# tomer-erez/Psychoacoustic-adverserial-attacks

Measured on AMD Instinct MI355X. Metric: pgd_steps_per_sec, higher is better.
Workload: dtype bf16x3 (split-bf16 hi+lo, three MFMA passes, f32 accumulate: fp32-parity); 1 GPU; untargeted PGD, norm_type snr snr_db 40, Wav2Vec2-base (rule-generated weights), 32x10s 16 kHz clips per GPU, 150-token labels; global_batch=32, per_gpu_batch=32, samples_per_clip=160000, parallelism=dp1, hip_graph=True, hip_graph_replayed_steps=80

## Files before the change

psychoacoustic-adverserial-attacks_amd/build_ext.py:

```python
from __future__ import annotations

import hashlib
import os
import subprocess
import sys
from concurrent.futures import ThreadPoolExecutor

HERE = os.path.dirname(os.path.abspath(__file__))
CSRC = os.path.join(HERE, "csrc")
INCLUDE = os.path.join(os.path.dirname(HERE), "include")
SOURCES = ["proj_kernels.hip", "spec_kernels.hip", "mask_kernels.hip", "gemm.hip", "gemm_ring.hip", "gemm_ring2.hip", "model_kernels.hip", "conv0_dgrad.hip", "attention.hip", "model.hip", "wer_kernels.hip", "place_kernels.hip", "rir_kernels.hip", "chan_kernels.hip", "search_kernels.hip", "eot_kernels.hip"]
FLAGS = ["-O3", "--offload-arch=gfx950", "-fPIC", "-std=c++17", "-Wno-unused-value"] + os.environ.get("PAA_EXTRA_HIPCC_FLAGS", "").split()
VARIANT = "_exp" if os.environ.get("PAA_EXTRA_HIPCC_FLAGS", "").strip() else ""
LIB = os.path.join(HERE, f"libpaa_hip{VARIANT}.so")


def _hipcc() -> str:
    for c in (os.environ.get("HIPCC"), "/opt/rocm/bin/hipcc", "hipcc"):
        if c and (os.path.isabs(c) and os.path.exists(c) or not os.path.isabs(c)):
            return c
    return "hipcc"


def _digest(paths, extra=()) -> str:
    h = hashlib.sha256()
    for x in extra:
        h.update(str(x).encode() + b"\0")
    for p in sorted(paths):
        h.update(os.path.basename(p).encode() + b"\0")
        with open(p, "rb") as f:
            h.update(f.read())
        h.update(b"\0")
    return h.hexdigest()


def _headers():
    out = [os.path.join(CSRC, f) for f in os.listdir(CSRC) if f.endswith(".h")]
    out += [os.path.join(INCLUDE, f) for f in os.listdir(INCLUDE) if f.endswith(".h")]
    return out


def source_key() -> str:
    files = [os.path.join(CSRC, f) for f in os.listdir(CSRC) if f.endswith((".hip", ".h"))]
    files += [os.path.join(INCLUDE, f) for f in os.listdir(INCLUDE) if f.endswith(".h")]
    return _digest(files, FLAGS + SOURCES)


def _read(path):
    try:
        with open(path) as f:
            return f.read().strip()
    except OSError:
        return None


def is_current() -> bool:
    return os.path.exists(LIB) and _read(LIB + ".key") == source_key()


def build(force: bool = False, verbose: bool = True) -> str:
    key = source_key()
    if not force and os.path.exists(LIB) and _read(LIB + ".key") == key:
        return LIB
    objdir = os.path.join(HERE, "build" + VARIANT)
    os.makedirs(objdir, exist_ok=True)
    hipcc = _hipcc()
    hdrs = _headers()

    def cc(src):
        obj = os.path.join(objdir, src.replace(".hip", ".o"))
        okey = _digest([os.path.join(CSRC, src)] + hdrs, FLAGS)
        if not force and os.path.exists(obj) and _read(obj + ".key") == okey:
            return obj
        cmd = [hipcc, *FLAGS, "-c", os.path.join(CSRC, src), "-o", obj]
        if verbose:
            print(" ".join(cmd), flush=True)
        r = subprocess.run(cmd, capture_output=True, text=True)
        if r.returncode != 0:
            raise RuntimeError(f"hipcc failed on {src}:\n{r.stdout}\n{r.stderr}")
        with open(obj + ".key", "w") as f:
            f.write(okey)
        return obj

    with ThreadPoolExecutor(max_workers=4) as ex:
        objs = list(ex.map(cc, SOURCES))
    cmd = [hipcc, "--offload-arch=gfx950", "-shared", "-fPIC", "-o", LIB, *objs]
    if verbose:
        print(" ".join(cmd), flush=True)
    r = subprocess.run(cmd, capture_output=True, text=True)
    if r.returncode != 0:
        raise RuntimeError(f"link failed:\n{r.stdout}\n{r.stderr}")
    with open(LIB + ".key", "w") as f:
        f.write(key)
    return LIB


if __name__ == "__main__":
    print(build(force="--force" in sys.argv))
```

psychoacoustic-adverserial-attacks_amd/csrc/gemm.hip:

```cpp
#include <algorithm>
#include <vector>

#include "gemm_dev.h"

namespace paa {

template <int ROWS, bool IS_A>
__device__ __forceinline__ void load_kc(const paa_gemm_desc& d, const float* __restrict__ base, int64_t ld, int r0,
                                        int k0, int rlim, float4 (&v)[ROWS / 32]) {
    const int tid = threadIdx.x;
    const int k = k0 + ((tid & 7) << 2);
    int64_t koff = k;
    int js = 0, kc = k;
    if (IS_A && d.a_kseg > 0) {
        js = k / d.a_kseg;
        kc = k - js * d.a_kseg;
        koff = (int64_t)js * d.a_kseg_stride + kc;
    }
#pragma unroll
    for (int i = 0; i < ROWS / 32; ++i) {
        const int r = r0 + (tid >> 3) + 32 * i;
        float4 x = make_float4(0.f, 0.f, 0.f, 0.f);
        bool ok = (r < rlim) && (k < d.K);
        const float* p;
        if (IS_A && d.a_window) {
            const int tr = r + js - d.a_pad;
            ok = ok && (tr >= 0) && (tr < d.a_rows_valid);
            p = base + (int64_t)tr * ld + kc;
        } else {
            p = base + (int64_t)r * ld + koff;
        }
        if (ok) {
            x = *reinterpret_cast<const float4*>(p);
            if (k + 3 >= d.K) {
                if (k + 1 >= d.K) x.y = 0.f;
                if (k + 2 >= d.K) x.z = 0.f;
                x.w = 0.f;
            }
        }
        v[i] = x;
    }
}

template <int ROWS>
__device__ __forceinline__ void load_rc(const paa_gemm_desc& d, const float* __restrict__ base, int64_t ld, int r0,
                                        int k0, int rlim, float4 (&v)[ROWS / 32]) {
    constexpr int VPK = ROWS / 4;
    constexpr int KSTEP = G_NT / VPK;
    const int tid = threadIdx.x;
    const int r = r0 + ((tid % VPK) << 2);
#pragma unroll
    for (int i = 0; i < ROWS / 32; ++i) {
        const int k = k0 + tid / VPK + KSTEP * i;
        float4 x = make_float4(0.f, 0.f, 0.f, 0.f);
        if (k < d.K && r < rlim) {
            x = *reinterpret_cast<const float4*>(base + (int64_t)k * ld + r);
            if (r + 3 >= rlim) {
                if (r + 1 >= rlim) x.y = 0.f;
                if (r + 2 >= rlim) x.z = 0.f;
                x.w = 0.f;
            }
        }
        v[i] = x;
    }
}

template <int ROWS, int PREC>
__device__ __forceinline__ void store_kc(unsigned short* hi, unsigned short* lo, const float4 (&v)[ROWS / 32]) {
    const int tid = threadIdx.x;
#pragma unroll
    for (int i = 0; i < ROWS / 32; ++i) {
        const int off = ((tid >> 3) + 32 * i) * G_LD + ((tid & 7) << 2);
        const float f[4] = {v[i].x, v[i].y, v[i].z, v[i].w};
        unsigned short h[4], l[4];
#pragma unroll
        for (int j = 0; j < 4; ++j) {
            h[j] = bf16_bits(f[j]);
            if (PREC) l[j] = bf16_bits(f[j] - bf16_to_f32(h[j]));
        }
        *reinterpret_cast<uint2*>(hi + off) = make_uint2(h[0] | ((unsigned)h[1] << 16), h[2] | ((unsigned)h[3] << 16));
        if (PREC)
            *reinterpret_cast<uint2*>(lo + off) = make_uint2(l[0] | ((unsigned)l[1] << 16), l[2] | ((unsigned)l[3] << 16));
    }
}

template <int ROWS, int PREC>
__device__ __forceinline__ void store_rc(unsigned short* hi, unsigned short* lo, const float4 (&v)[ROWS / 32]) {
    constexpr int VPK = ROWS / 4;
    constexpr int KSTEP = G_NT / VPK;
    const int tid = threadIdx.x;
#pragma unroll
    for (int i = 0; i < ROWS / 32; ++i) {
        const int k = tid / VPK + KSTEP * i;
        const int r = (tid % VPK) << 2;
        const float f[4] = {v[i].x, v[i].y, v[i].z, v[i].w};
#pragma unroll
        for (int j = 0; j < 4; ++j) {
            const unsigned short h = bf16_bits(f[j]);
            hi[(r + j) * G_LD + k] = h;
            if (PREC) lo[(r + j) * G_LD + k] = bf16_bits(f[j] - bf16_to_f32(h));
        }
    }
}

template <int BN, int PREC, bool AKC, bool BKC>
__global__ __launch_bounds__(G_NT) void k_gemm(GemmArgs g) {
    constexpr int NPL = PREC ? 2 : 1;
    constexpr int NJ = BN / 64;
    __shared__ __attribute__((aligned(16))) unsigned short smem[NPL * (G_BM + BN) * G_LD];
    unsigned short* sAh = smem;
    unsigned short* sAl = smem + (PREC ? G_BM * G_LD : 0);
    unsigned short* sBh = smem + NPL * G_BM * G_LD;
    unsigned short* sBl = sBh + (PREC ? BN * G_LD : 0);

    const paa_gemm_desc& d = g.d;
    const int nwg = g.tiles_m * g.tiles_n;
    const int orig = blockIdx.x;
    const int q = nwg >> 3, r8 = nwg & 7, xcd = orig & 7;
    const int id = (xcd < r8 ? xcd * (q + 1) : r8 * (q + 1) + (xcd - r8) * q) + (orig >> 3);
    const int tm = id / g.tiles_n, tn = id - tm * g.tiles_n;
    const int m0 = tm * G_BM, n0 = tn * BN;
    const int z = blockIdx.y;
    const int z1 = z / d.batch2, z2 = z - z1 * d.batch2;
    const float* A = d.A + z1 * d.a_s1 + z2 * d.a_s2;
    const float* B = d.B + z1 * d.b_s1 + z2 * d.b_s2;

    const int tid = threadIdx.x, lane = tid & 63, wave = tid >> 6;
    const int wm = wave >> 1, wn = wave & 1;
    const int lr = lane & 31, lh = lane >> 5;

    f32x16 acc[2][NJ];
#pragma unroll
    for (int i = 0; i < 2; ++i)
#pragma unroll
        for (int j = 0; j < NJ; ++j)
#pragma unroll
            for (int e = 0; e < 16; ++e) acc[i][j][e] = 0.f;

    float4 ra[G_BM / 32], rb[BN / 32];
    const int nk = (d.K + G_BK - 1) / G_BK;
    if (AKC) load_kc<G_BM, true>(d, A, d.lda, m0, 0, d.M, ra); else load_rc<G_BM>(d, A, d.lda, m0, 0, d.M, ra);
    if (BKC) load_kc<BN, false>(d, B, d.ldb, n0, 0, d.N, rb); else load_rc<BN>(d, B, d.ldb, n0, 0, d.N, rb);

    for (int kt = 0; kt < nk; ++kt) {
        if (AKC) store_kc<G_BM, PREC>(sAh, sAl, ra); else store_rc<G_BM, PREC>(sAh, sAl, ra);
        if (BKC) store_kc<BN, PREC>(sBh, sBl, rb); else store_rc<BN, PREC>(sBh, sBl, rb);
        __syncthreads();
        if (kt + 1 < nk) {
            const int k0 = (kt + 1) * G_BK;
            if (AKC) load_kc<G_BM, true>(d, A, d.lda, m0, k0, d.M, ra); else load_rc<G_BM>(d, A, d.lda, m0, k0, d.M, ra);
            if (BKC) load_kc<BN, false>(d, B, d.ldb, n0, k0, d.N, rb); else load_rc<BN>(d, B, d.ldb, n0, k0, d.N, rb);
        }
#pragma unroll
        for (int ks = 0; ks < 2; ++ks) {
            bf16x8 ah[2], al[2], bh[NJ], bl[NJ];
#pragma unroll
            for (int i = 0; i < 2; ++i) {
                const int off = (wm * 64 + i * 32 + lr) * G_LD + ks * 16 + lh * 8;
                ah[i] = *reinterpret_cast<const bf16x8*>(sAh + off);
                if (PREC) al[i] = *reinterpret_cast<const bf16x8*>(sAl + off);
            }
#pragma unroll
            for (int j = 0; j < NJ; ++j) {
                const int off = (wn * (BN / 2) + j * 32 + lr) * G_LD + ks * 16 + lh * 8;
                bh[j] = *reinterpret_cast<const bf16x8*>(sBh + off);
                if (PREC) bl[j] = *reinterpret_cast<const bf16x8*>(sBl + off);
            }
#pragma unroll
            for (int i = 0; i < 2; ++i)
#pragma unroll
                for (int j = 0; j < NJ; ++j) {
                    if (PREC) {
                        acc[i][j] = __builtin_amdgcn_mfma_f32_32x32x16_bf16(al[i], bh[j], acc[i][j], 0, 0, 0);
                        acc[i][j] = __builtin_amdgcn_mfma_f32_32x32x16_bf16(ah[i], bl[j], acc[i][j], 0, 0, 0);
                    }
                    acc[i][j] = __builtin_amdgcn_mfma_f32_32x32x16_bf16(ah[i], bh[j], acc[i][j], 0, 0, 0);
                }
        }
        __syncthreads();
    }

    epilogue<NJ, 2>(d, acc, m0 + wm * 64 + 4 * lh, n0 + wn * (BN / 2) + lr, z1, z2);
}

constexpr int H_BK = 64, H_LD = 72;

template <int ROWS, bool IS_A, int NT>
__device__ __forceinline__ void load_bf(const paa_gemm_desc& d, const unsigned short* __restrict__ base, int64_t ld,
                                        int r0, int k0, int rlim, uint4 (&v)[ROWS * 8 / NT], int tid, int il = 0) {
    const int k = k0 + ((tid & 7) << 3);
    int64_t koff = il ? ((k >> 5) << 6) + (k & 31) + (il == 2 ? 32 : 0) : k;
    int js = 0, kc = k;
    if (IS_A && d.a_kseg > 0) {
        js = k / d.a_kseg;
        kc = k - js * d.a_kseg;
        koff = (int64_t)js * d.a_kseg_stride + kc;
    }
#pragma unroll
    for (int i = 0; i < ROWS * 8 / NT; ++i) {
        const int r = r0 + (tid >> 3) + (NT / 8) * i;
        uint4 x = make_uint4(0u, 0u, 0u, 0u);
        bool ok = (r < rlim) && (k < d.K);
        const unsigned short* p;
        if (IS_A && d.a_window) {
            const int tr = r + js - d.a_pad;
            ok = ok && (tr >= 0) && (tr < d.a_rows_valid);
            p = base + (int64_t)tr * ld + kc;
        } else {
            p = base + (int64_t)r * ld + koff;
        }
        if (ok) x = *reinterpret_cast<const uint4*>(p);
        v[i] = x;
    }
}

typedef unsigned int u32x4 __attribute__((ext_vector_type(4)));
__device__ __forceinline__ __amdgpu_buffer_rsrc_t tile_rsrc(const unsigned short* base, int64_t elems) {
    const int64_t bytes = elems > 0 ? 2 * elems : 0;
    return __builtin_amdgcn_make_buffer_rsrc(const_cast<unsigned short*>(base), 0,
                                             (int)(unsigned)(bytes > 0xFFFFFFFFll ? 0xFFFFFFFFll : bytes), 0x00020000);
}
template <int ROWS, int NT>
__device__ __forceinline__ void load_buf(__amdgpu_buffer_rsrc_t rs, unsigned voff, unsigned k0_bytes, unsigned step_bytes,
                                         uint4 (&v)[ROWS * 8 / NT]) {
#pragma unroll
    for (int i = 0; i < ROWS * 8 / NT; ++i) {
        const u32x4 x = __builtin_amdgcn_raw_buffer_load_b128(rs, voff, k0_bytes + i * step_bytes, 0);
        v[i] = make_uint4(x.x, x.y, x.z, x.w);
    }
}

template <int ROWS, int NT, bool PERM, bool SWZ = false>
__device__ __forceinline__ void store_bf(unsigned short* lds, const uint4 (&v)[ROWS * 8 / NT], int tid) {
    constexpr int LD = SWZ ? 64 : H_LD;
#pragma unroll
    for (int i = 0; i < ROWS * 8 / NT; ++i) {
        int r = (tid >> 3) + (NT / 8) * i;
        if (PERM) r = (r & ~63) | ((((r >> 2) & 1) << 5) + (((r & 63) >> 3) << 2) + (r & 3));
        const int ch = SWZ ? ((tid & 7) ^ ((r >> 1) & 7)) : (tid & 7);
        *reinterpret_cast<uint4*>(lds + r * LD + (ch << 3)) = v[i];
    }
}

template <int BM, int BN, int PREC, int WM, bool VEC, bool SEG, bool SWZ = false>
__global__ __launch_bounds__(WM * 128, (WM == 4 && PREC == 0) ? 4 : 2) void k_gemm_bf(GemmArgs g) {
    constexpr int NT = WM * 128;
    constexpr int LD = SWZ ? 64 : H_LD;
    constexpr int NPL = PREC ? 2 : 1;
    constexpr int NJ = BN / 64;
    constexpr int MI = BM / (32 * WM);
    static_assert(!VEC || NJ == 2, "vector epilogue needs 64 columns per wave");
    __shared__ __attribute__((aligned(16))) unsigned short smem[NPL * (BM + BN) * LD];
    unsigned short* sAh = smem;
    unsigned short* sAl = smem + (PREC ? BM * LD : 0);
    unsigned short* sBh = smem + NPL * BM * LD;
    unsigned short* sBl = sBh + (PREC ? BN * LD : 0);

    const paa_gemm_desc& d = g.d;
    const int nwg = g.tiles_m * g.tiles_n;
    const int total = nwg * d.batch;
    const int nk = (d.K + H_BK - 1) / H_BK;
    const int kg_spt = (d.k_group > 0 && d.k_group % H_BK == 0 && d.K % d.k_group == 0 && d.K > d.k_group) ? d.k_group / H_BK : 0;
    const int kg_taps = kg_spt ? d.K / d.k_group : 1;

    struct Tile { int m0, n0, z1, z2; };
    auto decode = [&](int t) {
        Tile c;
        const int z = t / nwg, orig = t - z * nwg;
        const int q = nwg >> 3, r8 = nwg & 7, xcd = orig & 7;
        const int id = (xcd < r8 ? xcd * (q + 1) : r8 * (q + 1) + (xcd - r8) * q) + (orig >> 3);
        const int tm = id / g.tiles_n, tn = id - tm * g.tiles_n;
        c.m0 = tm * BM; c.n0 = tn * BN;
        c.z1 = z / d.batch2; c.z2 = z - c.z1 * d.batch2;
        return c;
    };
    uint4 rah[BM * 8 / NT], rbh[BN * 8 / NT], ral[PREC ? BM * 8 / NT : 1], rbl[PREC ? BN * 8 / NT : 1];
    auto load_tile = [&](const Tile& c, int k0, int tid) {
        const int64_t aoff = c.z1 * d.a_s1 + c.z2 * d.a_s2, boff = c.z1 * d.b_s1 + c.z2 * d.b_s2;
        if constexpr (SEG) {
            const bool ail = PREC && d.A_il != nullptr;
            if (ail) load_bf<BM, true, NT>(d, reinterpret_cast<const unsigned short*>(d.A_il) + 2 * aoff, 2 * d.lda, c.m0, k0, d.M, rah, tid, 1);
            else load_bf<BM, true, NT>(d, reinterpret_cast<const unsigned short*>(d.A) + aoff, d.lda, c.m0, k0, d.M, rah, tid);
            load_bf<BN, false, NT>(d, reinterpret_cast<const unsigned short*>(d.B) + boff, d.ldb, c.n0, k0, d.N, rbh, tid);
            if constexpr (PREC) {
                if (ail) load_bf<BM, true, NT>(d, reinterpret_cast<const unsigned short*>(d.A_il) + 2 * aoff, 2 * d.lda, c.m0, k0, d.M, ral, tid, 2);
                else load_bf<BM, true, NT>(d, reinterpret_cast<const unsigned short*>(d.A_lo) + aoff, d.lda, c.m0, k0, d.M, ral, tid);
                load_bf<BN, false, NT>(d, reinterpret_cast<const unsigned short*>(d.B_lo) + boff, d.ldb, c.n0, k0, d.N, rbl, tid);
            }
        } else if (PREC && d.A_il != nullptr) {
            const int64_t a0 = 2 * aoff + (int64_t)c.m0 * (2 * d.lda), b0 = boff + (int64_t)c.n0 * d.ldb;
            const int64_t ae = (int64_t)(d.M - 1 - c.m0) * (2 * d.lda) + 2 * (int64_t)d.K, be = (int64_t)(d.N - 1 - c.n0) * d.ldb + d.K;
            const unsigned kc = (unsigned)((tid & 7) << 3);
            const unsigned va = 2u * ((unsigned)(tid >> 3) * 2u * (unsigned)d.lda + ((kc >> 5) << 6) + (kc & 31u)), vb = 2u * ((unsigned)(tid >> 3) * (unsigned)d.ldb + kc);
            const unsigned sa = 2u * (NT / 8) * 2u * (unsigned)d.lda, sb = 2u * (NT / 8) * (unsigned)d.ldb;
            const __amdgpu_buffer_rsrc_t ra = tile_rsrc(reinterpret_cast<const unsigned short*>(d.A_il) + a0, ae);
            load_buf<BM, NT>(ra, va, 4u * k0, sa, rah);
            load_buf<BN, NT>(tile_rsrc(reinterpret_cast<const unsigned short*>(d.B) + b0, be), vb, 2u * k0, sb, rbh);
            if constexpr (PREC) {
                load_buf<BM, NT>(ra, va + 64u, 4u * k0, sa, ral);
                load_buf<BN, NT>(tile_rsrc(reinterpret_cast<const unsigned short*>(d.B_lo) + b0, be), vb, 2u * k0, sb, rbl);
            }
        } else {
            const int64_t a0 = aoff + (int64_t)c.m0 * d.lda, b0 = boff + (int64_t)c.n0 * d.ldb;
            const int64_t ae = (int64_t)(d.M - 1 - c.m0) * d.lda + d.K, be = (int64_t)(d.N - 1 - c.n0) * d.ldb + d.K;
            const unsigned kc = (unsigned)((tid & 7) << 3);
            const unsigned va = 2u * ((unsigned)(tid >> 3) * (unsigned)d.lda + kc), vb = 2u * ((unsigned)(tid >> 3) * (unsigned)d.ldb + kc);
            const unsigned sa = 2u * (NT / 8) * (unsigned)d.lda, sb = 2u * (NT / 8) * (unsigned)d.ldb;
            load_buf<BM, NT>(tile_rsrc(reinterpret_cast<const unsigned short*>(d.A) + a0, ae), va, 2u * k0, sa, rah);
            load_buf<BN, NT>(tile_rsrc(reinterpret_cast<const unsigned short*>(d.B) + b0, be), vb, 2u * k0, sb, rbh);
            if constexpr (PREC) {
                load_buf<BM, NT>(tile_rsrc(reinterpret_cast<const unsigned short*>(d.A_lo) + a0, ae), va, 2u * k0, sa, ral);
                load_buf<BN, NT>(tile_rsrc(reinterpret_cast<const unsigned short*>(d.B_lo) + b0, be), vb, 2u * k0, sb, rbl);
            }
        }
    };
    auto store_tile = [&](int tid) {
        store_bf<BM, NT, false, SWZ>(sAh, rah, tid);
        store_bf<BN, NT, VEC, SWZ>(sBh, rbh, tid);
        if constexpr (PREC) { store_bf<BM, NT, false, SWZ>(sAl, ral, tid); store_bf<BN, NT, VEC, SWZ>(sBl, rbl, tid); }
    };

    int t = blockIdx.x;
    if (t >= total) return;
    Tile cur = decode(t);
    load_tile(cur, 0, threadIdx.x);
    store_tile(threadIdx.x);
    for (;;) {
        int tid = threadIdx.x;
        asm volatile("" : "+v"(tid));
        const int lane = tid & 63, wave = tid >> 6;
        const int wm = wave >> 1, wn = wave & 1;
        const int lr = lane & 31, lh = lane >> 5;
        const int tnx = t + gridDim.x;
        const bool more = tnx < total;
        const Tile nxt = more ? decode(tnx) : cur;
        f32x16 acc[MI][NJ];
#pragma unroll
        for (int i = 0; i < MI; ++i)
#pragma unroll
            for (int j = 0; j < NJ; ++j)
#pragma unroll
                for (int e = 0; e < 16; ++e) acc[i][j][e] = 0.f;

        int ktap = 0, kc = 0;
        for (int kt = 0; kt < nk; ++kt) {
            __syncthreads();
            const bool last = kt + 1 == nk;
            int knext = kt + 1;
            if (kg_spt) {
                if (++ktap == kg_taps) { ktap = 0; ++kc; }
                knext = ktap * kg_spt + kc;
            }
            if (!last) load_tile(cur, knext * H_BK, tid);
            else if (more) load_tile(nxt, 0, tid);
            {
                constexpr int KS = H_BK / 16;
                constexpr int NM = NJ * (PREC ? 3 : 1);
                int offk[KS];
#pragma unroll
                for (int q = 0; q < KS; ++q) offk[q] = SWZ ? (((2 * q + lh) ^ ((lr >> 1) & 7)) << 3) : (lh * 8 + q * 16);
                const unsigned short* pa = sAh + (wm * (32 * MI) + lr) * LD;
                const unsigned short* pb = sBh + (wn * (BN / 2) + lr) * LD;
                constexpr int LO_A = BM * LD, LO_B = BN * LD;
                bf16x8 bh[NJ], bl[NJ], bhn[NJ], bln[NJ], ah, al, ahn, aln;
#pragma unroll
                for (int j = 0; j < NJ; ++j) {
                    bh[j] = *reinterpret_cast<const bf16x8*>(pb + j * 32 * LD + offk[0]);
                    if (PREC) bl[j] = *reinterpret_cast<const bf16x8*>(pb + LO_B + j * 32 * LD + offk[0]);
                    bhn[j] = bh[j]; bln[j] = bl[j];
                }
                ah = *reinterpret_cast<const bf16x8*>(pa + offk[0]);
                if (PREC) al = *reinterpret_cast<const bf16x8*>(pa + LO_A + offk[0]);
                ahn = ah; aln = al;
                __builtin_amdgcn_sched_group_barrier(0x100, (NJ + 1) * NPL, 0);
#pragma unroll
                for (int ks = 0; ks < KS; ++ks)
#pragma unroll
                    for (int i = 0; i < MI; ++i) {
                        const int ni = (i + 1 < MI) ? i + 1 : 0, nks = (i + 1 < MI) ? ks : ks + 1;
                        if (nks < KS) {
                            ahn = *reinterpret_cast<const bf16x8*>(pa + ni * 32 * LD + offk[nks < KS ? nks : 0]);
                            if (PREC) aln = *reinterpret_cast<const bf16x8*>(pa + LO_A + ni * 32 * LD + offk[nks < KS ? nks : 0]);
                            if (ni == 0) {
#pragma unroll
                                for (int j = 0; j < NJ; ++j) {
                                    bhn[j] = *reinterpret_cast<const bf16x8*>(pb + j * 32 * LD + offk[nks < KS ? nks : 0]);
                                    if (PREC) bln[j] = *reinterpret_cast<const bf16x8*>(pb + LO_B + j * 32 * LD + offk[nks < KS ? nks : 0]);
                                }
                            }
                        }
#pragma unroll
                        for (int j = 0; j < NJ; ++j) {
                            if (PREC) {
                                acc[i][j] = __builtin_amdgcn_mfma_f32_32x32x16_bf16(al, bh[j], acc[i][j], 0, 0, 0);
                                acc[i][j] = __builtin_amdgcn_mfma_f32_32x32x16_bf16(ah, bl[j], acc[i][j], 0, 0, 0);
                            }
                            acc[i][j] = __builtin_amdgcn_mfma_f32_32x32x16_bf16(ah, bh[j], acc[i][j], 0, 0, 0);
                        }
                        if (nks < KS) {
                            if (ni == 0) __builtin_amdgcn_sched_group_barrier(0x100, (NJ + 1) * NPL, 0);
                            else __builtin_amdgcn_sched_group_barrier(0x100, NPL, 0);
                        }
                        __builtin_amdgcn_sched_group_barrier(0x008, NM, 0);
                        ah = ahn; al = aln;
                        if (ni == 0) {
#pragma unroll
                            for (int j = 0; j < NJ; ++j) { bh[j] = bhn[j]; bl[j] = bln[j]; }
                        }
                    }
            }
            __syncthreads();
            if (!last || more) store_tile(tid);
        }
        {
            int te = tid;
            asm volatile("" : "+v"(te));
            const int el = te & 63, ew = te >> 6;
            if constexpr (VEC) epilogue_vec<MI, true>(d, acc, cur.m0 + (ew >> 1) * (32 * MI), cur.n0 + (ew & 1) * (BN / 2), cur.z1, cur.z2, el);
            else epilogue<NJ, MI>(d, acc, cur.m0 + (ew >> 1) * (32 * MI) + 4 * (el >> 5), cur.n0 + (ew & 1) * (BN / 2) + (el & 31), cur.z1, cur.z2);
        }
        if (!more) break;
        cur = nxt;
        t = tnx;
    }
}

template <int PREC, int KS, int MI, int WV = 4>
__global__ __launch_bounds__(WV * 64, WV == 4 ? 2 : 1) void k_gemm_win(GemmArgs g, int taps) {
    constexpr int NT = WV * 64;
    constexpr int BM = 32 * MI * WV, TB = 4, NPL = PREC ? 2 : 1;
    constexpr int ALD = KS + 8;
    constexpr int BLD = TB * KS + 8;
    constexpr int CPR = KS / 8;
    constexpr int BCH = TB * KS / 8;
    constexpr int NB = (64 * BCH + NT - 1) / NT;
    extern __shared__ __attribute__((aligned(16))) unsigned short smw[];
    const paa_gemm_desc& d = g.d;
    const int srows = BM + taps - 1;
    unsigned short* sA = smw;
    unsigned short* sB = smw + NPL * srows * ALD;
    const int tid = threadIdx.x, lane = tid & 63, wave = tid >> 6, lr = lane & 31, lh = lane >> 5;
    const int m0 = blockIdx.x * BM;
    const int z = blockIdx.y, z1 = z / d.batch2, z2 = z - z1 * d.batch2;
    const int64_t aoff = z1 * d.a_s1 + z2 * d.a_s2, boff = z1 * d.b_s1 + z2 * d.b_s2;
    const unsigned short* Ap[2] = {reinterpret_cast<const unsigned short*>(d.A) + aoff,
                                   PREC ? reinterpret_cast<const unsigned short*>(d.A_lo) + aoff : nullptr};
    const unsigned short* Bp[2] = {reinterpret_cast<const unsigned short*>(d.B) + boff,
                                   PREC ? reinterpret_cast<const unsigned short*>(d.B_lo) + boff : nullptr};
    for (int i = tid; i < srows * CPR; i += NT) {
        const int sr = i / CPR, ch = i - sr * CPR;
        const int tr = m0 - d.a_pad + sr;
        const bool ok = tr >= 0 && tr < d.a_rows_valid;
#pragma unroll
        for (int pl = 0; pl < NPL; ++pl) {
            uint4 x = make_uint4(0u, 0u, 0u, 0u);
            if (ok) x = *reinterpret_cast<const uint4*>(Ap[pl] + (int64_t)tr * d.lda + ch * 8);
            *reinterpret_cast<uint4*>(sA + (pl * srows + sr) * ALD + ch * 8) = x;
        }
    }
    for (int i = tid; i < NPL * 64 * BLD / 8; i += NT) reinterpret_cast<uint4*>(sB)[i] = make_uint4(0u, 0u, 0u, 0u);
    uint4 rb[NPL][NB];
    auto bload = [&](int st) {
#pragma unroll
        for (int u = 0; u < NB; ++u) {
            const int i = tid + NT * u;
            const int n = i / BCH, ch = i - n * BCH;
#pragma unroll
            for (int pl = 0; pl < NPL; ++pl) {
                rb[pl][u] = make_uint4(0u, 0u, 0u, 0u);
                if (i < 64 * BCH && n < d.N) rb[pl][u] = *reinterpret_cast<const uint4*>(Bp[pl] + (int64_t)n * d.ldb + st * (TB * KS) + ch * 8);
            }
        }
    };
    auto bstore = [&]() {
#pragma unroll
        for (int u = 0; u < NB; ++u) {
            const int i = tid + NT * u;
            const int n = i / BCH, ch = i - n * BCH;
            if (i < 64 * BCH && n < d.N) {
#pragma unroll
                for (int pl = 0; pl < NPL; ++pl) *reinterpret_cast<uint4*>(sB + (pl * 64 + n) * BLD + ch * 8) = rb[pl][u];
            }
        }
    };
    __syncthreads();
    bload(0);
    bstore();
    f32x16 acc[MI][2];
#pragma unroll
    for (int i = 0; i < MI; ++i)
#pragma unroll
        for (int j = 0; j < 2; ++j)
#pragma unroll
            for (int e = 0; e < 16; ++e) acc[i][j][e] = 0.f;
    const int nst = taps / TB;
    for (int st = 0; st < nst; ++st) {
        __syncthreads();
        if (st + 1 < nst) bload(st + 1);
        constexpr int NSTEP = TB * (KS / 16);
        const unsigned short* pa0 = sA + (wave * (32 * MI) + lr + st * TB) * ALD + lh * 8;
        const unsigned short* pb0 = sB + lr * BLD + lh * 8;
        bf16x8 ah[2][MI], al[2][MI], bh[2][2], bl[2][2];
        auto fload = [&](int q, int buf) {
            const int tp = q / (KS / 16), ks = q - tp * (KS / 16);
            const unsigned short* pa = pa0 + tp * ALD + ks * 16;
            const unsigned short* pb = pb0 + tp * KS + ks * 16;
#pragma unroll
            for (int i = 0; i < MI; ++i) {
                ah[buf][i] = *reinterpret_cast<const bf16x8*>(pa + i * 32 * ALD);
                if (PREC) al[buf][i] = *reinterpret_cast<const bf16x8*>(pa + (srows + i * 32) * ALD);
            }
#pragma unroll
            for (int j = 0; j < 2; ++j) {
                bh[buf][j] = *reinterpret_cast<const bf16x8*>(pb + j * 32 * BLD);
                if (PREC) bl[buf][j] = *reinterpret_cast<const bf16x8*>(pb + (64 + j * 32) * BLD);
            }
        };
        fload(0, 0);
#pragma unroll
        for (int q = 0; q < NSTEP; ++q) {
            const int cb = q & 1;
            if (q + 1 < NSTEP) fload(q + 1, cb ^ 1);
#pragma unroll
            for (int j = 0; j < 2; ++j)
#pragma unroll
                for (int i = 0; i < MI; ++i) {
                    if (PREC) {
                        acc[i][j] = __builtin_amdgcn_mfma_f32_32x32x16_bf16(al[cb][i], bh[cb][j], acc[i][j], 0, 0, 0);
                        acc[i][j] = __builtin_amdgcn_mfma_f32_32x32x16_bf16(ah[cb][i], bl[cb][j], acc[i][j], 0, 0, 0);
                    }
                    acc[i][j] = __builtin_amdgcn_mfma_f32_32x32x16_bf16(ah[cb][i], bh[cb][j], acc[i][j], 0, 0, 0);
                }
            if constexpr (PREC == 0) {
#pragma unroll
                for (int r = 0; r < (MI + 2 > 2 * MI ? MI + 2 : 2 * MI); ++r) {
                    if (r < 2 * MI) __builtin_amdgcn_sched_group_barrier(0x008, 1, 0);
                    if (r < MI + 2 && q + 1 < NSTEP) __builtin_amdgcn_sched_group_barrier(0x100, 1, 0);
                }
            }
        }
        __syncthreads();
        if (st + 1 < nst) bstore();
    }
    epilogue<2, MI>(d, acc, m0 + wave * (32 * MI) + 4 * lh, lr, z1, z2);
}

template <int BM, int BN, int PREC, int WM, bool VEC, bool SEG, bool SWZ = false>
static void launch_bf(const GemmArgs& g, hipStream_t st) {
    static const int per_cu = blocks_per_cu(k_gemm_bf<BM, BN, PREC, WM, VEC, SEG, SWZ>, WM * 128);
    const int resident = per_cu * device_cus();
    const int total = g.tiles_m * g.tiles_n * g.d.batch;
    const int blocks = resident > 0 ? std::min(total, resident) : total;
    hipLaunchKernelGGL((k_gemm_bf<BM, BN, PREC, WM, VEC, SEG, SWZ>), dim3(blocks), dim3(WM * 128), 0, st, g);
}

void launch_ring_cfg(int cfg, const GemmArgs& g, hipStream_t st);
void launch_ring2_cfg(int cfg, const GemmArgs& g, hipStream_t st);
int ring_tile_rows(int cfg);
int ring_tile_cols(int cfg);
bool ring_cfg_ok(int cfg, const paa_gemm_desc& d, bool forced = false);

static int g_ring_mode = 0;
struct GemmEnv { bool init = false, no_sq = false, no_r2 = false, kgroup = true, no_bil = false; };
static GemmEnv g_env;
static void gemm_env_refresh() {
#ifdef PAA_EXPERIMENTS
    auto on = [](const char* name, char v) { const char* e = getenv(name); return e && e[0] == v; };
    g_env.no_sq = on("PAA_NO_SQ", '1');
    g_env.no_r2 = on("PAA_NO_R2", '1');
    g_env.kgroup = !on("PAA_K_GROUP", '0');
    g_env.no_bil = on("PAA_NO_BIL", '1');
#endif
    g_env.init = true;
}
bool gemm_env_no_bil() {
    if (!g_env.init) gemm_env_refresh();
    return g_env.no_bil;
}
bool gemm_env_kgroup() {
    if (!g_env.init) gemm_env_refresh();
    return g_env.kgroup;
}

static int g_last_kind = EPK_GENERIC;
static int classify_epilogue(const paa_gemm_desc& d) {
#ifdef PAA_EXPERIMENTS
    { const char* e = getenv("PAA_NO_EPIK"); if (e && e[0] == '1') return EPK_GENERIC; }
#endif
    if (d.alpha != 1.f || d.accumulate || d.aux_bf16 || !d.precision) return EPK_GENERIC;
    const bool il = d.Cb_il && !d.Cb && !d.Cb_lo, planar = d.Cb && d.Cb_lo && !d.Cb_il, no_planes = !d.Cb && !d.Cb_lo && !d.Cb_il;
    const bool mask = d.row_period > 0;
    switch (d.act) {
        case PAA_ACT_GELU:
            return (d.bias && d.C_pre && d.aux_gate && il && !d.C && !d.aux && !d.residual && !d.res_ln_stats) ? EPK_GELU_FWD : EPK_GENERIC;
        case PAA_ACT_GELU_GRAD:
            if (!(d.aux && d.aux_gate && (il || planar) && !d.bias && !d.C && !d.C_pre && !d.residual && !d.res_ln_stats && !mask)) return EPK_GENERIC;
#ifdef PAA_EXPERIMENTS
            { const char* e = getenv("PAA_EPIK_AHEAD"); if (e && e[0] == '2') return EPK_GELU_GRAD_LA2; if (e && e[0] == '4') return EPK_GELU_GRAD_LA4; }
#endif
            return EPK_GELU_GRAD;
        case PAA_ACT_NONE:
            if (d.C_pre || d.aux || d.aux_gate || mask) return EPK_GENERIC;
            if (d.C && no_planes && d.residual) {
                if (d.res_ln_stats) return d.bias ? EPK_RESID_LN : EPK_GENERIC;
                return d.bias ? EPK_GENERIC : EPK_RESID;
            }
            if (!d.C && planar && !d.residual && !d.res_ln_stats) return EPK_PLANES;
            return EPK_GENERIC;
        default: return EPK_GENERIC;
    }
}

template <int BN, int PREC>
static void launch_gemm(const GemmArgs& g, dim3 grid, hipStream_t st) {
    const bool akc = g.d.a_kcontig != 0, bkc = g.d.b_kcontig != 0;
    if (akc && bkc) hipLaunchKernelGGL((k_gemm<BN, PREC, true, true>), grid, dim3(G_NT), 0, st, g);
    else if (akc && !bkc) hipLaunchKernelGGL((k_gemm<BN, PREC, true, false>), grid, dim3(G_NT), 0, st, g);
    else if (!akc && bkc) hipLaunchKernelGGL((k_gemm<BN, PREC, false, true>), grid, dim3(G_NT), 0, st, g);
    else hipLaunchKernelGGL((k_gemm<BN, PREC, false, false>), grid, dim3(G_NT), 0, st, g);
}

struct GemmProf {
    bool on = false;
    std::vector<hipEvent_t> ev;
    std::vector<double> flops, bytes;
    std::vector<int> variant;
    size_t n = 0, cap = 0;
};
static GemmProf g_prof;

paa_status gemm(const paa_gemm_desc& d, hipStream_t st) {
    if ((!d.A && !d.A_il) || !d.B || (!d.C && !d.Cb && !d.Cb_il)) PAA_FAIL(PAA_ERR_ARG, "gemm: null operand");
    if (d.A_il) {
        if (!d.precision || !d.operand_bf16 || d.a_kseg > 0 || d.a_window || (d.lda & 31) || (d.K & 31) || (d.a_s1 & 31) || (d.a_s2 & 31) || ((uintptr_t)d.A_il & 15))
            PAA_FAIL(PAA_ERR_ARG, "gemm: A_il needs split precision, plain K-contiguous bf16 rows and lda / K / batch strides that are multiples of 32");
    }
    if (d.Cb_il) {
        if (!d.precision || d.Cb || d.Cb_lo || (d.ldc & 31) || (d.c_s1 & 31) || (d.c_s2 & 31) || ((uintptr_t)d.Cb_il & 15))
            PAA_FAIL(PAA_ERR_ARG, "gemm: Cb_il needs split precision, no Cb / Cb_lo, and ldc / batch strides that are multiples of 32");
    }
    if (d.accumulate && !d.C) PAA_FAIL(PAA_ERR_ARG, "gemm: accumulate needs the f32 result");
    if (d.Cb_lo && !d.Cb) PAA_FAIL(PAA_ERR_ARG, "gemm: Cb_lo without Cb");
    if (d.M <= 0 || d.N <= 0 || d.K <= 0 || d.batch <= 0 || d.batch2 <= 0) PAA_FAIL(PAA_ERR_SIZE, "gemm: bad dims %d %d %d", d.M, d.N, d.K);
    const int al = d.operand_bf16 ? 7 : 3;
    if ((d.lda & al) || (d.ldb & al) || (!d.A_il && ((uintptr_t)d.A & 15)) || ((uintptr_t)d.B & 15))
        PAA_FAIL(PAA_ERR_ARG, "gemm: operands must be 16-byte aligned with leading dimensions that are multiples of %d", al + 1);
    if ((d.a_s1 & al) || (d.a_s2 & al) || (d.b_s1 & al) || (d.b_s2 & al)) PAA_FAIL(PAA_ERR_ARG, "gemm: batch strides must be multiples of %d", al + 1);
    if (d.a_kseg > 0 && ((d.a_kseg & al) || (d.a_kseg_stride & al) || !d.a_kcontig)) PAA_FAIL(PAA_ERR_ARG, "gemm: bad K segmentation");
    if (d.operand_bf16) {
        if (!d.a_kcontig || !d.b_kcontig || (d.K & 7)) PAA_FAIL(PAA_ERR_ARG, "gemm: bf16 operands must be K-contiguous with K %% 8 == 0 (K=%d)", d.K);
        if (d.precision && ((!d.A_il && (!d.A_lo || ((uintptr_t)d.A_lo & 15))) || !d.B_lo || ((uintptr_t)d.B_lo & 15)))
            PAA_FAIL(PAA_ERR_ARG, "gemm: split precision needs aligned lo planes");
    }
    if (d.a_window && d.a_kseg <= 0) PAA_FAIL(PAA_ERR_ARG, "gemm: a_window needs a_kseg");
    if (d.act == PAA_ACT_GELU_GRAD && !d.aux) PAA_FAIL(PAA_ERR_ARG, "gemm: GELU_GRAD needs aux");
    if (d.res_ln_stats && (!d.residual || !d.res_ln_g || !d.res_ln_b || d.batch != 1 || d.act == PAA_ACT_GELU_GRAD ||
                           ((uintptr_t)d.res_ln_stats & 7) || ((uintptr_t)d.res_ln_g & 15) || ((uintptr_t)d.res_ln_b & 15)))
        PAA_FAIL(PAA_ERR_ARG, "gemm: res_ln_stats needs a residual, gain and bias (16-byte aligned), batch 1 and no GELU_GRAD");
    GemmArgs g;
    g.d = d;
    g.kind = EPK_GENERIC;
    const bool narrow = d.N <= 64;
    const int bn = narrow ? 64 : 128;
    auto al16 = [](const void* p) { return ((uintptr_t)p & 15) == 0; };
    const bool vec = d.operand_bf16 && !narrow && (d.N & 7) == 0 && (d.ldc & 7) == 0 && (d.c_s1 & 7) == 0 && (d.c_s2 & 7) == 0 &&
                     al16(d.C) && al16(d.C_pre) && al16(d.Cb) && al16(d.Cb_lo) && al16(d.Cb_il) &&
                     (!d.aux || (al16(d.aux) && (d.ld_aux & (d.aux_bf16 ? 7 : 3)) == 0 && (d.aux_s1 & 7) == 0 && (d.aux_s2 & 7) == 0)) &&
                     (!d.residual || (al16(d.residual) && (d.ld_res & 3) == 0 && (d.res_s1 & 3) == 0 && (d.res_s2 & 3) == 0)) &&
                     (!d.bias || (al16(d.bias) && (d.bias_s2 & 3) == 0)) &&
                     !(d.act == PAA_ACT_GELU_GRAD && d.residual) &&
                     63 * d.lda < (1ll << 30) && 63 * d.ldb < (1ll << 30) && (int64_t)d.M * d.ldc < (1ll << 30) && (int64_t)d.M * std::max(d.ld_aux, d.ld_res) < (1ll << 30);
    const bool tall = vec && d.a_kseg <= 0 && (d.K & 63) == 0 && d.M >= 2048;
    bool bm192 = false;
    if (tall && !d.precision) {
        static const int per_cu = std::max(1, blocks_per_cu(k_gemm_bf<256, 128, 0, 2, true, false>, 256));
        const int slots = per_cu * device_cus();
        const int64_t tn = cdiv(d.N, 128);
        const int64_t t256 = (int64_t)cdiv(d.M, 256) * tn * d.batch, t192 = (int64_t)cdiv(d.M, 192) * tn * d.batch;
        const double c256 = (double)((t256 + slots - 1) / slots) * 256.0, c192 = (double)((t192 + slots - 1) / slots) * 192.0 * 1.05;
        bm192 = c192 < c256;
    }
    int ring = 0;
    const bool forced2 = g_ring_mode >= 20 && vec && d.a_kseg <= 0 && ring_cfg_ok(g_ring_mode, d, true);
    if ((tall || forced2) && g_ring_mode != 1 && d.N >= 128) {
        const int64_t t256 = (int64_t)cdiv(d.M, 256) * cdiv(d.N, 256) * d.batch, t128 = (int64_t)cdiv(d.M, 256) * cdiv(d.N, 128) * d.batch;
        if (!g_env.init) gemm_env_refresh();
        const bool no_sq = g_env.no_sq;
        if (g_ring_mode >= 2) ring = g_ring_mode;
        else if (d.precision) {
            const int64_t slots = device_cus();
            const int64_t r256 = (t128 + slots - 1) / slots;
            const int64_t t192 = (int64_t)cdiv(d.M, 192) * cdiv(d.N, 128) * d.batch;
            const int64_t r192 = (t192 + 2 * slots - 1) / (2 * slots);
            const int64_t rsq = (t256 + slots - 1) / slots;
            const double c256 = (double)r256 * 256.0, c192 = (double)r192 * 192.0 * 2.0 / 0.95, csq = (double)rsq * 512.0 / 1.08;
            ring = 0;
            double best = c256;
            if (c192 < best && !d.A_il) { best = c192; ring = 7; }
            if (!no_sq && d.N % 256 == 0 && ring_cfg_ok(20, d) && csq < best) { best = csq; ring = 20; }
            const int64_t r18 = ((int64_t)cdiv(d.M, 192) * cdiv(d.N, 256) * d.batch + slots - 1) / slots;
            const double c18 = (double)r18 * 384.0 / 1.05;
            if (!no_sq && d.N % 256 == 0 && ring_cfg_ok(22, d) && c18 < best) { best = c18; ring = 22; }
        } else if (bm192) {
            ring = 8;
            const int64_t cus = device_cus();
            const int64_t r8 = ((int64_t)cdiv(d.M, 192) * cdiv(d.N, 128) * d.batch + 2 * cus - 1) / (2 * cus), r19 = ((int64_t)cdiv(d.M, 192) * cdiv(d.N, 256) * d.batch + cus - 1) / cus;
            if (!no_sq && d.N % 256 == 0 && ring_cfg_ok(23, d) && r19 <= r8) ring = 23;
        } else if (!no_sq && d.N % 256 == 0 && ring_cfg_ok(21, d)) {
            static const int per_cu2 = std::max(1, blocks_per_cu(k_gemm_bf<256, 128, 0, 2, true, false>, 256));
            const int64_t cus = device_cus(), slots2 = per_cu2 * cus;
            const int64_t r2 = (t128 + slots2 - 1) / slots2, rsq = (t256 + cus - 1) / cus;
            if (rsq <= r2) ring = 21;
        }
#ifdef PAA_EXPERIMENTS
        if (g_ring_mode < 2 && g_env.no_r2 && ring >= 20) {
            const int r1 = ring == 20 ? 17 : ring == 21 ? 2 : ring == 22 ? 18 : 19;
            if (ring_cfg_ok(r1, d)) ring = r1;
        }
#endif
#ifdef PAA_EXPERIMENTS
        if (ring == 13) { if (!d.precision) ring = 0; }
        else
#endif
        if (ring && !ring_cfg_ok(ring, d, forced2)) ring = 0;
        if (ring && ring < 20 && d.A_il) ring = 0;
    }
    const int ring_bn = ring == 13 ? 128 : ring ? ring_tile_cols(ring) : 0, ring_bm = ring == 13 ? 192 : ring ? ring_tile_rows(ring) : 0;
    g.tiles_m = cdiv(d.M, ring ? ring_bm : tall ? (bm192 ? 192 : 256) : G_BM);
    g.tiles_n = cdiv(d.N, ring ? ring_bn : bn);
    dim3 grid(g.tiles_m * g.tiles_n, d.batch);
    const bool prof = g_prof.on && g_prof.n < g_prof.cap;
    if (prof) {
        (void)hipEventRecord(g_prof.ev[2 * g_prof.n], st);
        g_prof.flops[g_prof.n] = 2.0 * d.M * d.N * (double)d.K * d.batch;
        {
            const double es = d.operand_bf16 ? 2.0 * (d.precision ? 2 : 1) : 4.0;
            const double a_el = (d.a_kcontig && d.lda > 0 && d.lda < d.K && !d.a_window && d.a_kseg <= 0) ? ((double)(d.M - 1) * d.lda + d.K) : (double)d.M * d.K;
            const double mn = (double)d.M * d.N;
            double by = a_el * es + (double)d.N * d.K * es;
            if (d.a_window) by = (double)d.a_rows_valid * d.a_kseg * es + (double)d.N * d.K * es;
            if (d.C) by += mn * 4.0 * (d.accumulate ? 2 : 1);
            if (d.Cb) by += mn * 2.0 * (d.Cb_lo ? 2 : 1);
            if (d.Cb_il) by += mn * 4.0;
            if (d.C_pre) by += mn * (d.aux_bf16 ? 2.0 : 4.0);
            if (d.aux) by += mn * (d.aux_bf16 ? 2.0 : 4.0);
            if (d.residual) by += mn * 4.0;
            g_prof.bytes[g_prof.n] = by * d.batch;
        }
        g_prof.variant[g_prof.n] = (tall ? 32 : 0) + (d.operand_bf16 ? 16 : 0) + ((narrow || bm192) ? 8 : 0) + (d.precision ? 4 : 0) + (d.a_kcontig ? 2 : 0) + (d.b_kcontig ? 1 : 0);
    }
    if (d.operand_bf16 && d.a_window && (d.a_kseg == 48 || d.a_kseg == 64) && d.N <= 64 && d.K % (4 * d.a_kseg) == 0 &&
        d.ldb >= d.K && d.a_kseg_stride == d.lda) {
        const int taps = d.K / d.a_kseg;
        const int npl = d.precision ? 2 : 1;
        const int mi = (d.a_kseg == 48 && d.M > 128) ? 2 : 1;
        const size_t lds = 2 * (size_t)npl * ((size_t)(128 * mi + taps - 1) * (d.a_kseg + 8) + 64 * (size_t)(4 * d.a_kseg + 8));
        if (lds <= 150 * 1024) {
            dim3 wgrid(cdiv(d.M, 128 * mi), d.batch);
#define PAA_WIN(P, KS_, MI_, WV_)                                                                                            \
            {                                                                                                                \
                static bool attr = false;                                                                                    \
                if (!attr) { PAA_HIP(hipFuncSetAttribute(reinterpret_cast<const void*>(&k_gemm_win<P, KS_, MI_, WV_>), hipFuncAttributeMaxDynamicSharedMemorySize, 152 * 1024)); attr = true; } \
                hipLaunchKernelGGL((k_gemm_win<P, KS_, MI_, WV_>), wgrid, dim3(WV_ * 64), lds, st, g, taps);                 \
            }
            if (prof) { g_prof.variant[g_prof.n] = 40 + (d.precision ? 4 : 0); }
            if (d.a_kseg == 48) {
                if (mi == 2) { if (d.precision) PAA_WIN(1, 48, 1, 8) else PAA_WIN(0, 48, 2, 4) }
                else { if (d.precision) PAA_WIN(1, 48, 1, 4) else PAA_WIN(0, 48, 1, 4) }
            }
            else { if (d.precision) PAA_WIN(1, 64, 1, 4) else PAA_WIN(0, 64, 1, 4) }
#undef PAA_WIN
            if (prof) { (void)hipEventRecord(g_prof.ev[2 * g_prof.n + 1], st); ++g_prof.n; }
            PAA_LAUNCH_CHECK();
            return PAA_OK;
        }
    }
    if (ring) {
        if (prof) g_prof.variant[g_prof.n] = (ring_bm == 192 ? (ring_bn == 128 ? 60 : 52) : (ring_bn == 256 ? 56 : 48)) + (d.precision ? 1 : 0);
#ifdef PAA_EXPERIMENTS
        if (ring == 13) launch_bf<192, 128, 1, 2, true, false, true>(g, st);
        else
#endif
        if (ring >= 20) {
            g.kind = g_last_kind = classify_epilogue(d);
            int taken = 1 << EPK_GELU_FWD;
#ifdef PAA_EXPERIMENTS
            { const char* e = getenv("PAA_EPIK_MASK"); const int mask = e ? atoi(e) : 0; if (mask > 0) taken = mask; }
#endif
            if (!((taken >> g.kind) & 1)) g.kind = EPK_GENERIC;
            launch_ring2_cfg(ring, g, st);
        }
        else launch_ring_cfg(ring, g, st);
    } else if (d.operand_bf16) {
        const bool seg = d.a_kseg > 0 || (d.K & 63);
        if (narrow) {
            if (seg) { if (d.precision) launch_bf<128, 64, 1, 2, false, true>(g, st); else launch_bf<128, 64, 0, 2, false, true>(g, st); }
            else { if (d.precision) launch_bf<128, 64, 1, 2, false, false>(g, st); else launch_bf<128, 64, 0, 2, false, false>(g, st); }
        }
        else if (seg && vec && !d.precision) launch_bf<128, 128, 0, 2, true, true>(g, st);
        else if (seg) { if (d.precision) launch_bf<128, 128, 1, 2, false, true>(g, st); else launch_bf<128, 128, 0, 2, false, true>(g, st); }
        else if (tall) {
            if (d.precision) launch_bf<256, 128, 1, 4, true, false>(g, st);
            else if (bm192) launch_bf<192, 128, 0, 2, true, false>(g, st);
            else launch_bf<256, 128, 0, 2, true, false>(g, st);
        }
        else if (vec) { if (d.precision) launch_bf<128, 128, 1, 2, true, false>(g, st); else launch_bf<128, 128, 0, 2, true, false>(g, st); }
        else { if (d.precision) launch_bf<128, 128, 1, 2, false, false>(g, st); else launch_bf<128, 128, 0, 2, false, false>(g, st); }
    } else if (narrow) { if (d.precision) launch_gemm<64, 1>(g, grid, st); else launch_gemm<64, 0>(g, grid, st); }
    else { if (d.precision) launch_gemm<128, 1>(g, grid, st); else launch_gemm<128, 0>(g, grid, st); }
    if (prof) { (void)hipEventRecord(g_prof.ev[2 * g_prof.n + 1], st); ++g_prof.n; }
    PAA_LAUNCH_CHECK();
    return PAA_OK;
}

}

extern "C" paa_status paa_prof_enable(int max_launches) {
    using namespace paa;
    for (hipEvent_t e : g_prof.ev) (void)hipEventDestroy(e);
    g_prof.ev.clear(); g_prof.n = 0; g_prof.cap = 0; g_prof.on = false;
    if (max_launches <= 0) return PAA_OK;
    g_prof.ev.resize(2 * (size_t)max_launches);
    for (auto& e : g_prof.ev) PAA_HIP(hipEventCreate(&e));
    g_prof.flops.assign(max_launches, 0.0);
    g_prof.bytes.assign(max_launches, 0.0);
    g_prof.variant.assign(max_launches, 0);
    g_prof.cap = max_launches; g_prof.on = true;
    return PAA_OK;
}

extern "C" paa_status paa_prof_read(double* out256) {
    using namespace paa;
    if (!out256) PAA_FAIL(PAA_ERR_ARG, "paa_prof_read: null");
    for (int i = 0; i < 256; ++i) out256[i] = 0.0;
    if (g_prof.n == 0) return PAA_OK;
    PAA_HIP(hipEventSynchronize(g_prof.ev[2 * g_prof.n - 1]));
    for (size_t i = 0; i < g_prof.n; ++i) {
        float ms = 0.f;
        PAA_HIP(hipEventElapsedTime(&ms, g_prof.ev[2 * i], g_prof.ev[2 * i + 1]));
        const int v = g_prof.variant[i];
        out256[4 * v] += 1.0; out256[4 * v + 1] += ms; out256[4 * v + 2] += g_prof.flops[i]; out256[4 * v + 3] += g_prof.bytes[i];
    }
    g_prof.n = 0;
    return PAA_OK;
}

extern "C" paa_status paa_prof_pause(int paused) {
    paa::g_prof.on = !paused && paa::g_prof.cap > 0;
    return PAA_OK;
}

#ifdef PAA_EXPERIMENTS
extern "C" int paa_debug_last_epilogue_kind() { return paa::g_last_kind; }
#endif

extern "C" void paa_gemm_config(int ring_mode) { paa::g_ring_mode = ring_mode; paa::gemm_env_refresh(); }

extern "C" paa_status paa_gemm(const struct paa_gemm_desc* d, void* stream) {
    if (!d) { paa::set_error("paa_gemm: null descriptor"); return PAA_ERR_ARG; }
    return paa::gemm(*d, (hipStream_t)stream);
}
```

Baseline: 28.39 steps/s (one step = PGD step on 32 x 10 s clips; counted over all ranks).

## Add specialized thin-N and thin-K split-bf16 GEMM kernels

Adds a new source file with two register-only MFMA kernels for bf16x3 GEMMs whose N is at most 64 or K is at most 64. These shapes are routed away from the ring and tiled paths, which waste tile capacity on such skinny shapes. The thin-N kernel streams K with one wave per 32-row block, and the thin-K kernel keeps the A fragment in registers while waves sweep N chunks. The risks are low occupancy or uncoalesced B loads on large M, and that some epilogue features are left unsupported, so those cases still use the existing paths.

```diff
diff --git a/psychoacoustic-adverserial-attacks_amd/build_ext.py b/psychoacoustic-adverserial-attacks_amd/build_ext.py
--- a/psychoacoustic-adverserial-attacks_amd/build_ext.py
+++ b/psychoacoustic-adverserial-attacks_amd/build_ext.py
@@ -9,7 +9,7 @@
 HERE = os.path.dirname(os.path.abspath(__file__))
 CSRC = os.path.join(HERE, "csrc")
 INCLUDE = os.path.join(os.path.dirname(HERE), "include")
-SOURCES = ["proj_kernels.hip", "spec_kernels.hip", "mask_kernels.hip", "gemm.hip", "gemm_ring.hip", "gemm_ring2.hip", "model_kernels.hip", "conv0_dgrad.hip", "attention.hip", "model.hip", "wer_kernels.hip", "place_kernels.hip", "rir_kernels.hip", "chan_kernels.hip", "search_kernels.hip", "eot_kernels.hip"]
+SOURCES = ["proj_kernels.hip", "spec_kernels.hip", "mask_kernels.hip", "gemm.hip", "gemm_thin.hip", "gemm_ring.hip", "gemm_ring2.hip", "model_kernels.hip", "conv0_dgrad.hip", "attention.hip", "model.hip", "wer_kernels.hip", "place_kernels.hip", "rir_kernels.hip", "chan_kernels.hip", "search_kernels.hip", "eot_kernels.hip"]
 FLAGS = ["-O3", "--offload-arch=gfx950", "-fPIC", "-std=c++17", "-Wno-unused-value"] + os.environ.get("PAA_EXTRA_HIPCC_FLAGS", "").split()
 VARIANT = "_exp" if os.environ.get("PAA_EXTRA_HIPCC_FLAGS", "").strip() else ""
 LIB = os.path.join(HERE, f"libpaa_hip{VARIANT}.so")
diff --git a/psychoacoustic-adverserial-attacks_amd/csrc/gemm.hip b/psychoacoustic-adverserial-attacks_amd/csrc/gemm.hip
--- a/psychoacoustic-adverserial-attacks_amd/csrc/gemm.hip
+++ b/psychoacoustic-adverserial-attacks_amd/csrc/gemm.hip
@@ -559,6 +559,8 @@
 int ring_tile_rows(int cfg);
 int ring_tile_cols(int cfg);
 bool ring_cfg_ok(int cfg, const paa_gemm_desc& d, bool forced = false);
+int thin_kind(const paa_gemm_desc& d, bool vec);
+void launch_thin(int kind, const GemmArgs& g, hipStream_t st);
 
 static int g_ring_mode = 0;
 struct GemmEnv { bool init = false, no_sq = false, no_r2 = false, kgroup = true, no_bil = false; };
@@ -775,7 +777,9 @@
             return PAA_OK;
         }
     }
-    if (ring) {
+    const int thin = (g_ring_mode == 0 && !tall) ? thin_kind(d, vec) : 0;
+    if (thin) launch_thin(thin, g, st);
+    else if (ring) {
         if (prof) g_prof.variant[g_prof.n] = (ring_bm == 192 ? (ring_bn == 128 ? 60 : 52) : (ring_bn == 256 ? 56 : 48)) + (d.precision ? 1 : 0);
 #ifdef PAA_EXPERIMENTS
         if (ring == 13) launch_bf<192, 128, 1, 2, true, false, true>(g, st);
diff --git a/psychoacoustic-adverserial-attacks_amd/csrc/gemm_thin.hip b/psychoacoustic-adverserial-attacks_amd/csrc/gemm_thin.hip
--- /dev/null
+++ b/psychoacoustic-adverserial-attacks_amd/csrc/gemm_thin.hip
@@ -0,0 +1,148 @@
+#include "gemm_dev.h"
+
+namespace paa {
+
+struct ThinA {
+    const unsigned short* hi;
+    const unsigned short* lo;
+    bool il;
+    __device__ __forceinline__ int koff(int k) const { return il ? ((k >> 5) << 6) + (k & 31) : k; }
+};
+__device__ __forceinline__ ThinA thin_a(const paa_gemm_desc& d, int m0, int lr) {
+    const int r = min(m0 + lr, d.M - 1);
+    ThinA a;
+    a.il = d.A_il != nullptr;
+    if (a.il) {
+        a.hi = reinterpret_cast<const unsigned short*>(d.A_il) + (int64_t)r * (2 * d.lda);
+        a.lo = a.hi + 32;
+    } else {
+        a.hi = reinterpret_cast<const unsigned short*>(d.A) + (int64_t)r * d.lda;
+        a.lo = reinterpret_cast<const unsigned short*>(d.A_lo) + (int64_t)r * d.lda;
+    }
+    return a;
+}
+__device__ __forceinline__ bf16x8 ld8(const unsigned short* p) { return *reinterpret_cast<const bf16x8*>(p); }
+
+template <int NKS>
+__global__ __launch_bounds__(256) void k_gemm_thin_k(GemmArgs g) {
+    const paa_gemm_desc& d = g.d;
+    const int lane = threadIdx.x & 63, wave = threadIdx.x >> 6;
+    const int lr = lane & 31, lh = lane >> 5;
+    const int m0 = blockIdx.x * 32;
+    const ThinA a = thin_a(d, m0, lr);
+    bf16x8 ah[NKS], al[NKS];
+#pragma unroll
+    for (int ks = 0; ks < NKS; ++ks) {
+        const int ko = a.koff(ks * 16 + lh * 8);
+        ah[ks] = ld8(a.hi + ko);
+        al[ks] = ld8(a.lo + ko);
+    }
+    const unsigned short* Bh = reinterpret_cast<const unsigned short*>(d.B);
+    const unsigned short* Bl = reinterpret_cast<const unsigned short*>(d.B_lo);
+    const int nch = (d.N + 63) >> 6;
+    for (int ch = wave; ch < nch; ch += 4) {
+        const int n0 = ch * 64;
+        bf16x8 bh[2][NKS], bl[2][NKS];
+#pragma unroll
+        for (int j = 0; j < 2; ++j) {
+            const int n = min(n0 + 8 * (lr >> 2) + 4 * j + (lr & 3), d.N - 1);
+            const int64_t o = (int64_t)n * d.ldb + lh * 8;
+#pragma unroll
+            for (int ks = 0; ks < NKS; ++ks) {
+                bh[j][ks] = ld8(Bh + o + ks * 16);
+                bl[j][ks] = ld8(Bl + o + ks * 16);
+            }
+        }
+        f32x16 acc[1][2];
+#pragma unroll
+        for (int j = 0; j < 2; ++j)
+#pragma unroll
+            for (int e = 0; e < 16; ++e) acc[0][j][e] = 0.f;
+#pragma unroll
+        for (int ks = 0; ks < NKS; ++ks)
+#pragma unroll
+            for (int j = 0; j < 2; ++j) {
+                acc[0][j] = __builtin_amdgcn_mfma_f32_32x32x16_bf16(al[ks], bh[j][ks], acc[0][j], 0, 0, 0);
+                acc[0][j] = __builtin_amdgcn_mfma_f32_32x32x16_bf16(ah[ks], bl[j][ks], acc[0][j], 0, 0, 0);
+                acc[0][j] = __builtin_amdgcn_mfma_f32_32x32x16_bf16(ah[ks], bh[j][ks], acc[0][j], 0, 0, 0);
+            }
+        epilogue_vec<1, true>(d, acc, m0, n0, 0, 0, lane);
+    }
+}
+
+template <int NJ>
+__global__ __launch_bounds__(64) void k_gemm_thin_n(GemmArgs g) {
+    constexpr int U = 8;
+    const paa_gemm_desc& d = g.d;
+    const int lane = threadIdx.x, lr = lane & 31, lh = lane >> 5;
+    const int m0 = blockIdx.x * 32;
+    const ThinA a = thin_a(d, m0, lr);
+    const unsigned short* bhp[NJ];
+    const unsigned short* blp[NJ];
+#pragma unroll
+    for (int j = 0; j < NJ; ++j) {
+        const int64_t o = (int64_t)min(j * 32 + lr, d.N - 1) * d.ldb + lh * 8;
+        bhp[j] = reinterpret_cast<const unsigned short*>(d.B) + o;
+        blp[j] = reinterpret_cast<const unsigned short*>(d.B_lo) + o;
+    }
+    f32x16 acc[1][NJ];
+#pragma unroll
+    for (int j = 0; j < NJ; ++j)
+#pragma unroll
+        for (int e = 0; e < 16; ++e) acc[0][j][e] = 0.f;
+    const int nks = d.K >> 4;
+    for (int k0 = 0; k0 < nks; k0 += U) {
+        bf16x8 ah[U], al[U], bh[NJ][U], bl[NJ][U];
+#pragma unroll
+        for (int u = 0; u < U; ++u) {
+            if (k0 + u < nks) {
+                const int k = (k0 + u) * 16 + lh * 8;
+                const int ko = a.koff(k);
+                ah[u] = ld8(a.hi + ko);
+                al[u] = ld8(a.lo + ko);
+#pragma unroll
+                for (int j = 0; j < NJ; ++j) {
+                    bh[j][u] = ld8(bhp[j] + (k - lh * 8));
+                    bl[j][u] = ld8(blp[j] + (k - lh * 8));
+                }
+            }
+        }
+#pragma unroll
+        for (int u = 0; u < U; ++u) {
+            if (k0 + u < nks) {
+#pragma unroll
+                for (int j = 0; j < NJ; ++j) {
+                    acc[0][j] = __builtin_amdgcn_mfma_f32_32x32x16_bf16(al[u], bh[j][u], acc[0][j], 0, 0, 0);
+                    acc[0][j] = __builtin_amdgcn_mfma_f32_32x32x16_bf16(ah[u], bl[j][u], acc[0][j], 0, 0, 0);
+                    acc[0][j] = __builtin_amdgcn_mfma_f32_32x32x16_bf16(ah[u], bh[j][u], acc[0][j], 0, 0, 0);
+                }
+            }
+        }
+    }
+    epilogue<NJ, 1>(d, acc, m0 + 4 * lh, lr, 0, 0);
+}
+
+int thin_kind(const paa_gemm_desc& d, bool vec) {
+    if (!d.operand_bf16 || !d.precision || d.batch != 1 || d.a_kseg > 0 || d.a_window || d.k_group > 0 || (d.K & 15)) return 0;
+    if (d.N <= 64) return 2;
+    if (d.K <= 64 && vec && d.act == PAA_ACT_NONE && !d.res_ln_stats && !d.C_pre) return 1;
+    return 0;
+}
+
+void launch_thin(int kind, const GemmArgs& g, hipStream_t st) {
+    const dim3 grid(cdiv(g.d.M, 32));
+    if (kind == 1) {
+        switch (g.d.K >> 4) {
+            case 1: hipLaunchKernelGGL(k_gemm_thin_k<1>, grid, dim3(256), 0, st, g); break;
+            case 2: hipLaunchKernelGGL(k_gemm_thin_k<2>, grid, dim3(256), 0, st, g); break;
+            case 3: hipLaunchKernelGGL(k_gemm_thin_k<3>, grid, dim3(256), 0, st, g); break;
+            default: hipLaunchKernelGGL(k_gemm_thin_k<4>, grid, dim3(256), 0, st, g); break;
+        }
+    } else if (g.d.N <= 32) {
+        hipLaunchKernelGGL(k_gemm_thin_n<1>, grid, dim3(64), 0, st, g);
+    } else {
+        hipLaunchKernelGGL(k_gemm_thin_n<2>, grid, dim3(64), 0, st, g);
+    }
+}
+
+}
```

After: 28.47 steps/s (one step = PGD step on 32 x 10 s clips; counted over all ranks) (median of 6 runs). No clear change (+0.3%).
